# yang-song/score_sde_pytorch

Hardware: NVIDIA H100
Metric: PC-sampler images/sec, NCSN++ CIFAR-10 1000-step VE (higher is better)
Workload: dtype f16 operands (11-bit significand, as tf32), f32 accumulate and activations

## Files before the change

include/scoresde_b200.h:

```cpp
#ifndef SCORESDE_B200_H_
#define SCORESDE_B200_H_

#ifdef __cplusplus
extern "C" {
#endif

#define B200_API __attribute__((visibility("default")))

B200_API const char* b200_last_error(void);
B200_API int b200_version(void);
B200_API int b200_device_sm_count(int* out);

B200_API int b200_upfirdn2d_f32(const float* x, const float* kernel_host, float* y,
                                int major, int in_h, int in_w, int minor, int kh, int kw,
                                int up_x, int up_y, int down_x, int down_y,
                                int pad_x0, int pad_x1, int pad_y0, int pad_y1, void* stream);

B200_API int b200_fused_bias_act_f32(const float* x, const float* b, const float* ref, float* y,
                                     long long n, int step_b, int size_b, int act, int grad,
                                     float alpha, float scale, void* stream);

B200_API int b200_groupnorm_nhwc_f32(const float* x1, int c1, const float* x2, int c2,
                                     const float* gamma, const float* beta, int batch, int hw, int groups,
                                     float eps, int silu, int round_tf32,
                                     float* stats_ws ,
                                     float* y, float* raw_or_null, void* stream);
B200_API int b200_softmax_rows_f32(const float* s, float* p, long long rows, int t, float scale,
                                   int round_tf32, void* stream);
B200_API int b200_randn_like_torch_f32(float* out, long long numel, unsigned long long seed,
                                       unsigned long long offset, unsigned long long* offset_inc_out,
                                       unsigned long long* offset_ws_dev , void* stream);

B200_API int b200_conv_nhwc_f32(const float* x1, int c1, const float* x2, int c2, int batch, int h, int w,
                                const float* w_packed, const float* bias, int c_out, int ksize,
                                const float* rowvec, long long rowvec_ld, const float* residual, float scale,
                                int round_tf32, float* out, int impl, void* stream);
B200_API int b200_conv_skip_nhwc_f32(const float* x, int c, const float* s1, int cs1, const float* s2, int cs2,
                                     int batch, int h, int w, const float* w_packed, const float* bias,
                                     const float* w_skip, const float* bias_skip, int c_out, const float* residual,
                                     float scale, int round_tf32, float* out, void* stream);
B200_API int b200_pack_conv_weight_f32(const float* w_oihw, float* w_packed, int c_out, int c_in, int ksize,
                                       int round_tf32, void* stream);
B200_API int b200_attention_core_f32(const float* qk, const float* vT, const float* w3, const float* bv,
                                     const float* b3, const float* x, float* out, double* qstats, int nimg,
                                     int t, int c, float out_scale, int operand_f16, void* stream);
B200_API int b200_gemm_nt_f32(const float* a, long long lda, int a_batch_rows, const float* w, long long ldw,
                              int w_batch_rows, int nbatch, int m, int n, int k, const float* bias,
                              int round_tf32, float* out, long long ldo, int impl, void* stream);

typedef struct b200_ncsnpp b200_ncsnpp_t;

typedef struct {
  int image_size, num_channels, nf, num_res_blocks;
  int num_levels;  int ch_mult[8];
  int num_attn_resolutions;  int attn_resolutions[8];
  int centered, scale_by_sigma, skip_rescale, conditional;
  int progressive_input;
  int fir_taps;  float fir_kernel[8];
  int precision;
  int keep_activations;
  int lanes;
  int cuda_core_head;
  int separate_groupnorm;
  int embedding_type;
  int naive_resample;
  int progressive;
  int pdl;
  int no_halo;
  int family;
  int tangent;
} b200_ncsnpp_config;

B200_API int b200_ncsnpp_create(const b200_ncsnpp_config* cfg, b200_ncsnpp_t** out);
B200_API void b200_ncsnpp_destroy(b200_ncsnpp_t* h);
B200_API int b200_ncsnpp_num_params(const b200_ncsnpp_t* h);
B200_API int b200_ncsnpp_param_info(const b200_ncsnpp_t* h, int index, char* name, int name_cap,
                                    long long shape[4], int* ndim);
B200_API long long b200_ncsnpp_weights_bytes(const b200_ncsnpp_t* h);
B200_API int b200_ncsnpp_bind_weights(b200_ncsnpp_t* h, void* blob_dev);
B200_API int b200_ncsnpp_load_param(b200_ncsnpp_t* h, int index, const float* src_dev, void* stream);
B200_API long long b200_ncsnpp_workspace_bytes(b200_ncsnpp_t* h, int batch);
B200_API int b200_ncsnpp_bind_workspace(b200_ncsnpp_t* h, int batch, void* ws_dev, long long ws_bytes);
B200_API int b200_ncsnpp_forward(b200_ncsnpp_t* h, const float* x_nchw, const float* labels,
                                 int labels_uniform, float* out_nchw, void* stream);
B200_API int b200_ncsnpp_tap(b200_ncsnpp_t* h, int module_index, float* dst_nchw, long long dst_cap_elems,
                             int shape_out[4], void* stream);
B200_API long long b200_ncsnpp_launches_per_forward(const b200_ncsnpp_t* h);
B200_API int b200_ncsnpp_jvp(b200_ncsnpp_t* h, const float* x_nchw, const float* labels, int labels_uniform,
                             const float* v_nchw, float* out_nchw, float* jvp_out_nchw, void* stream);
B200_API int b200_ncsnpp_tap_tangent(b200_ncsnpp_t* h, int module_index, float* dst_nchw, long long dst_cap_elems,
                                     int shape_out[4], void* stream);
B200_API int b200_ncsnpp_profile_forward(b200_ncsnpp_t* h, const float* x_nchw, const float* labels,
                                         int labels_uniform, float* out_nchw, void* stream,
// ... 58 lines not shown
```

score_sde_pytorch_b200/_lib.py:

```python
import ctypes
import os
import threading

from . import build as _build

_LOCK = threading.Lock()
_LIB = None

c_void_p, c_int, c_ll, c_ull, c_float = (ctypes.c_void_p, ctypes.c_int, ctypes.c_longlong,
                                         ctypes.c_ulonglong, ctypes.c_float)
c_char_p = ctypes.c_char_p
P = ctypes.POINTER


class NcsnppConfig(ctypes.Structure):
  _fields_ = [('image_size', c_int), ('num_channels', c_int), ('nf', c_int), ('num_res_blocks', c_int),
              ('num_levels', c_int), ('ch_mult', c_int * 8),
              ('num_attn_resolutions', c_int), ('attn_resolutions', c_int * 8),
              ('centered', c_int), ('scale_by_sigma', c_int), ('skip_rescale', c_int), ('conditional', c_int),
              ('progressive_input', c_int),
              ('fir_taps', c_int), ('fir_kernel', c_float * 8),
              ('precision', c_int), ('keep_activations', c_int), ('lanes', c_int),
              ('cuda_core_head', c_int), ('separate_groupnorm', c_int),
              ('embedding_type', c_int), ('naive_resample', c_int), ('progressive', c_int), ('pdl', c_int),
              ('no_halo', c_int), ('family', c_int), ('tangent', c_int)]


class PcConfig(ctypes.Structure):
  _fields_ = [('n_steps', c_int), ('corrector', c_int), ('predictor', c_int), ('n_corrector_steps', c_int),
              ('snr', c_float),
              ('label', P(c_float)), ('score_scale', P(c_float)), ('alpha', P(c_float)),
              ('pa', P(c_float)), ('pb', P(c_float)), ('pc', P(c_float)),
              ('ca', P(c_float)), ('cb', P(c_float)), ('cc', P(c_float)),
              ('constraint', c_int), ('cm', P(c_float)), ('cs', P(c_float)),
              ('color_m', c_float * 9), ('color_minv', c_float * 9), ('noise_nhwc', c_int)]


SIGNATURES = {
  'b200_last_error': (c_char_p, []),
  'b200_version': (c_int, []),
  'b200_device_sm_count': (c_int, [P(c_int)]),
  'b200_upfirdn2d_f32': (c_int, [c_void_p, P(c_float), c_void_p] + [c_int] * 14 + [c_void_p]),
  'b200_fused_bias_act_f32': (c_int, [c_void_p, c_void_p, c_void_p, c_void_p, c_ll, c_int, c_int, c_int, c_int,
                                      c_float, c_float, c_void_p]),
  'b200_groupnorm_nhwc_f32': (c_int, [c_void_p, c_int, c_void_p, c_int, c_void_p, c_void_p, c_int, c_int, c_int,
                                      c_float, c_int, c_int, c_void_p, c_void_p, c_void_p, c_void_p]),
  'b200_softmax_rows_f32': (c_int, [c_void_p, c_void_p, c_ll, c_int, c_float, c_int, c_void_p]),
  'b200_randn_like_torch_f32': (c_int, [c_void_p, c_ll, c_ull, c_ull, P(c_ull), c_void_p, c_void_p]),
  'b200_conv_nhwc_f32': (c_int, [c_void_p, c_int, c_void_p, c_int, c_int, c_int, c_int, c_void_p, c_void_p, c_int,
                                 c_int, c_void_p, c_ll, c_void_p, c_float, c_int, c_void_p, c_int, c_void_p]),
  'b200_conv_skip_nhwc_f32': (c_int, [c_void_p, c_int, c_void_p, c_int, c_void_p, c_int, c_int, c_int, c_int, c_void_p,
                                      c_void_p, c_void_p, c_void_p, c_int, c_void_p, c_float, c_int, c_void_p, c_void_p]),
  'b200_attention_core_f32': (c_int, [c_void_p, c_void_p, c_void_p, c_void_p, c_void_p, c_void_p, c_void_p, c_void_p,
                                      c_int, c_int, c_int, c_float, c_int, c_void_p]),
  'b200_pack_conv_weight_f32': (c_int, [c_void_p, c_void_p, c_int, c_int, c_int, c_int, c_void_p]),
  'b200_gemm_nt_f32': (c_int, [c_void_p, c_ll, c_int, c_void_p, c_ll, c_int, c_int, c_int, c_int, c_int, c_void_p,
                               c_int, c_void_p, c_ll, c_int, c_void_p]),
  'b200_ncsnpp_create': (c_int, [P(NcsnppConfig), P(c_void_p)]),
  'b200_ncsnpp_destroy': (None, [c_void_p]),
  'b200_ncsnpp_num_params': (c_int, [c_void_p]),
  'b200_ncsnpp_param_info': (c_int, [c_void_p, c_int, c_char_p, c_int, P(c_ll), P(c_int)]),
  'b200_ncsnpp_weights_bytes': (c_ll, [c_void_p]),
  'b200_ncsnpp_bind_weights': (c_int, [c_void_p, c_void_p]),
  'b200_ncsnpp_load_param': (c_int, [c_void_p, c_int, c_void_p, c_void_p]),
  'b200_ncsnpp_num_ops': (c_ll, [c_void_p]),
  'b200_ncsnpp_op_info': (c_int, [c_void_p, c_ll, c_char_p, c_int, P(c_int), P(ctypes.c_double)]),
  'b200_ncsnpp_op_bytes': (c_int, [c_void_p, c_ll, P(ctypes.c_double)]),
  'b200_ncsnpp_profile_ops': (c_int, [c_void_p, c_void_p, c_void_p, c_int, c_void_p, c_void_p, c_void_p, c_ll]),
  'b200_ncsnpp_workspace_bytes': (c_ll, [c_void_p, c_int]),
  'b200_ncsnpp_bind_workspace': (c_int, [c_void_p, c_int, c_void_p, c_ll]),
  'b200_ncsnpp_forward': (c_int, [c_void_p, c_void_p, c_void_p, c_int, c_void_p, c_void_p]),
  'b200_ncsnpp_tap': (c_int, [c_void_p, c_int, c_void_p, c_ll, P(c_int), c_void_p]),
  'b200_ncsnpp_launches_per_forward': (c_ll, [c_void_p]),
  'b200_ncsnpp_jvp': (c_int, [c_void_p, c_void_p, c_void_p, c_int, c_void_p, c_void_p, c_void_p, c_void_p]),
  'b200_ncsnpp_tap_tangent': (c_int, [c_void_p, c_int, c_void_p, c_ll, P(c_int), c_void_p]),
  'b200_ncsnpp_profile_forward': (c_int, [c_void_p, c_void_p, c_void_p, c_int, c_void_p, c_void_p,
                                          P(c_float), P(ctypes.c_double), P(c_ll)]),
  'b200_pc_create': (c_int, [c_void_p, P(PcConfig), c_int, P(c_void_p)]),
  'b200_pc_destroy': (None, [c_void_p]),
  'b200_pc_workspace_bytes': (c_ll, [c_void_p]),
  'b200_pc_bind_workspace': (c_int, [c_void_p, c_void_p, c_ll, c_void_p]),
  'b200_pc_run': (c_int, [c_void_p, c_void_p, c_void_p, c_int, c_int, c_ull, c_ull, P(c_ull), c_int, c_void_p]),
  'b200_pc_bind_constraint': (c_int, [c_void_p, c_void_p, c_void_p, c_void_p]),
  'b200_pc_step_external': (c_int, [c_void_p, c_void_p, c_void_p, c_int, c_void_p, c_void_p, c_void_p]),
  'b200_pc_launches_per_step': (c_ll, [c_void_p]),
  'b200_ode_stage_f64': (c_int, [c_void_p, c_void_p, c_ll, P(ctypes.c_double), c_int, ctypes.c_double, c_void_p, c_void_p, c_void_p]),
  'b200_ode_drift_f64': (c_int, [c_void_p, c_void_p, c_ll, c_void_p, c_void_p, c_void_p]),
  'b200_ode_div_f64': (c_int, [c_void_p, c_void_p, c_int, c_ll, c_void_p, c_void_p, c_void_p]),
  'b200_ode_workspace_doubles': (c_ll, []),
  'b200_ode_error_sumsq_f64': (c_int, [c_void_p, c_void_p, c_void_p, c_ll, P(ctypes.c_double), c_int, ctypes.c_double,
                                       ctypes.c_double, ctypes.c_double, c_void_p, c_void_p]),
  'b200_ode_scaled_sumsq_f64': (c_int, [c_void_p, c_void_p, c_void_p, c_ll, ctypes.c_double, ctypes.c_double, c_void_p, c_void_p]),
  'b200_dsm_perturb_f32': (c_int, [c_void_p, c_void_p, c_void_p, c_void_p, c_void_p, c_int, c_ll, c_void_p]),
  'b200_dsm_workspace_doubles': (c_ll, [c_int, c_ll]),
  'b200_dsm_loss_f32': (c_int, [c_void_p, c_void_p, c_void_p, c_void_p, c_void_p, c_int, c_ll, c_int, c_int, c_void_p, c_void_p]),
}


def library_path():
  return _build.LIB


def load():
  global _LIB
  with _LOCK:
# ... 32 lines not shown
```

score_sde_pytorch_b200/csrc/api.cu:

```cuda
#include "kernels.h"
#include "../../include/scoresde_b200.h"
#include <cstring>

namespace b200 {
namespace { thread_local bool tl_pdl = false; }
bool pdl_active() { return tl_pdl; }
PdlScope::PdlScope(bool on) : prev(tl_pdl) { tl_pdl = on; }
PdlScope::~PdlScope() { tl_pdl = prev; }


static thread_local char g_err[1024] = "";

void set_error(const char* fmt, ...) {
  va_list ap;
  va_start(ap, fmt);
  vsnprintf(g_err, sizeof(g_err), fmt, ap);
  va_end(ap);
}
const char* last_error() { return g_err; }

}

using namespace b200;

// ... 63 lines not shown
}

int b200_conv_nhwc_f32(const float* x1, int c1, const float* x2, int c2, int batch, int h, int w,
                       const float* w_packed, const float* bias, int c_out, int ksize, const float* rowvec,
                       long long rowvec_ld, const float* residual, float scale, int round_tf32, float* out, int impl,
                       void* stream) {
  B200_REQUIRE(x1 && w_packed && out, "conv_nhwc: null pointer");
  B200_REQUIRE(ksize == 1 || ksize == 3, "conv_nhwc: ksize %d unsupported", ksize);
  cudaStream_t st = static_cast<cudaStream_t>(stream);
  Epilogue ep; memset(&ep, 0, sizeof(ep));
  ep.bias = bias; ep.rowvec = rowvec; ep.rowvec_ld = rowvec_ld; ep.residual = residual; ep.ld_res = c_out;
  ep.scale = scale; ep.round_tf32 = round_tf32; ep.rows_per_img = h * w; ep.out = out; ep.ld_out = c_out;
  if (!x2) c2 = 0;
  if (impl == 1 || impl == 2 || impl == 4 || impl == 5) {
    TcGemmDesc d; memset(&d, 0, sizeof(d));
    d.f16 = impl == 2 || impl == 5; d.no_halo = impl >= 4 ? 1 : 0;
    d.a1 = x1; d.C1 = c1; d.a2 = x2; d.C2 = c2; d.conv = 1; d.H = h; d.W = w; d.nimg = batch; d.taps = ksize * ksize;
    d.w = w_packed; d.N_total = c_out; d.K_total = c1 + c2; d.w_rows = (long long)ksize * ksize * c_out; d.nbatch = 1;
    d.epi = ep;
    TcGemmPlan* pl = nullptr;
    if (int r = tc_gemm_plan_create(d, &pl)) return r;
    const int r = tc_gemm_launch(pl, st);
    tc_gemm_plan_destroy(pl);
    return r;
  }
  SimtConv s; memset(&s, 0, sizeof(s));
  s.x1 = x1; s.C1 = c1; s.x2 = x2; s.C2 = c2; s.in_scale = 1.f; s.H = h; s.W = w; s.R = s.S = ksize; s.stride = 1;
  s.pad = ksize / 2; s.OH = h; s.OW = w; s.nbatch = batch; s.a_batched = 1; s.w = w_packed; s.N = c_out; s.epi = ep;
  if (impl == 3) return launch_conv_lowc(s, st);
  B200_REQUIRE(impl == 0, "conv_nhwc: impl %d unknown", impl);
  return launch_conv_simt(s, st);
}

int b200_conv_skip_nhwc_f32(const float* x, int c, const float* s1, int cs1, const float* s2, int cs2, int batch, int h,
                            int w, const float* w_packed, const float* bias, const float* w_skip,
                            const float* bias_skip, int c_out, const float* residual, float scale, int round_tf32,
                            float* out, void* stream) {
  B200_REQUIRE(x && s1 && w_packed && w_skip && out, "conv_skip_nhwc: null pointer");
  Epilogue ep; memset(&ep, 0, sizeof(ep));
  ep.bias = bias; ep.rowvec = bias_skip; ep.rowvec_ld = 0; ep.residual = residual; ep.ld_res = c_out;
  ep.scale = scale; ep.round_tf32 = round_tf32; ep.rows_per_img = h * w; ep.out = out; ep.ld_out = c_out;
  TcGemmDesc d; memset(&d, 0, sizeof(d));
  d.a1 = x; d.C1 = c; d.conv = 1; d.H = h; d.W = w; d.nimg = batch; d.taps = 9;
  d.w = w_packed; d.N_total = c_out; d.K_total = c; d.w_rows = 9LL * c_out; d.nbatch = 1;
  d.a3 = s1; d.C3 = cs1; d.a4 = s2; d.C4 = s2 ? cs2 : 0; d.w2 = w_skip;
  d.epi = ep;
  TcGemmPlan* pl = nullptr;
  if (int r = tc_gemm_plan_create(d, &pl)) return r;
  const int r = tc_gemm_launch(pl, static_cast<cudaStream_t>(stream));
  tc_gemm_plan_destroy(pl);
  return r;
}

int b200_attention_core_f32(const float* qk, const float* vT, const float* w3, const float* bv, const float* b3,
                            const float* x, float* out, double* qstats, int nimg, int t, int c, float out_scale,
                            int operand_f16, void* stream) {
  B200_REQUIRE(tc_attn_supported(t, c), "attention_core: only T=256, C=256 is implemented (got T=%d C=%d)", t, c);
  TcAttnDesc d; memset(&d, 0, sizeof(d));
  d.qk = qk; d.vT = vT; d.w3 = w3; d.bv = bv; d.b3 = b3; d.x = x; d.out = out; d.qstats = qstats;
  d.nimg = nimg; d.T = t; d.C = c; d.out_scale = out_scale; d.f16 = operand_f16 ? 1 : 0;
  TcAttnPlan* pl = nullptr;
  if (int r = tc_attn_plan_create(d, &pl)) return r;
  const int r = tc_attn_launch(pl, static_cast<cudaStream_t>(stream));
  tc_attn_plan_destroy(pl);
  return r;
}

int b200_gemm_nt_f32(const float* a, long long lda, int a_batch_rows, const float* w, long long ldw, int w_batch_rows,
                     int nbatch, int m, int n, int k, const float* bias, int round_tf32, float* out, long long ldo,
                     int impl, void* stream) {
  B200_REQUIRE(a && w && out && nbatch > 0, "gemm_nt: bad argument");
  cudaStream_t st = static_cast<cudaStream_t>(stream);
  Epilogue ep; memset(&ep, 0, sizeof(ep));
  ep.bias = bias; ep.scale = 1.f; ep.round_tf32 = round_tf32; ep.rows_per_img = m; ep.out = out; ep.ld_out = ldo;
  if (impl == 1 || impl == 2) {
    TcGemmDesc d; memset(&d, 0, sizeof(d));
    d.f16 = impl == 2;
    d.a1 = a; d.C1 = k; d.conv = 0; d.taps = 1; d.a_ld = lda; d.a_batch_rows = a_batch_rows;
    d.a_rows = a_batch_rows ? (long long)a_batch_rows * (nbatch - 1) + m : m;
    d.w = w; d.N_total = n; d.K_total = k; d.w_ld = ldw; d.w_batch_rows = w_batch_rows;
    d.w_rows = w_batch_rows ? (long long)w_batch_rows * (nbatch - 1) + n : n;
    d.nbatch = nbatch; d.M_per_batch = m; d.epi = ep;
    TcGemmPlan* pl = nullptr;
    if (int r = tc_gemm_plan_create(d, &pl)) return r;
    const int r = tc_gemm_launch(pl, st);
    tc_gemm_plan_destroy(pl);
    return r;
  }
  SimtConv s; memset(&s, 0, sizeof(s));
  s.x1 = a; s.C1 = k; s.ld1 = lda; s.in_scale = 1.f; s.H = m; s.W = 1; s.R = s.S = 1; s.stride = 1; s.pad = 0;
  s.OH = m; s.OW = 1; s.nbatch = nbatch; s.a_batched = a_batch_rows != 0; s.w = w; s.N = n;
  s.w_batch_stride = (long long)w_batch_rows * ldw; s.w_ld = ldw; s.epi = ep;
  B200_REQUIRE(!a_batch_rows || a_batch_rows == m, "gemm_nt(simt): a_batch_rows must be 0 or m");
  return launch_conv_simt(s, st);
}

}
```

score_sde_pytorch_b200/csrc/gemm_tc.cu:

```cuda
#include "kernels.h"
#include <cuda.h>
#include <cudaTypedefs.h>
#include <cuda_fp16.h>
#include "wgmma.cuh"
#include <mutex>
#include <cstdlib>
#include <cstring>

namespace b200 {

namespace {

constexpr int BM = 128;
constexpr int BKE = 32;
constexpr int A_STAGE_BYTES = BM * BKE * 4;

constexpr int HALO_XS = 4;
constexpr int HALO_X_BYTES = 40 * 1024;
constexpr int HALO_WS = 4;

struct TcParams {
  CUtensorMap tmA1, tmA2, tmW;
  CUtensorMap tmA3, tmA4, tmW2;
  CUtensorMap tmH1, tmH2;
  int halo;
  int halo_dh_bytes;
  int halo_copy_bytes;
  int halo_prefetch;
  int chunk_major;
  int conv, H, W, taps, pad, S, stride;
  int kchunks1, kchunks2, C1;
  int kchunks3, kchunks4, C3;
  int N_total, tiles_n;
  int nbatch, tiles_m_per_batch, M_per_batch;
  int a_batch_rows, w_batch_rows;
  int f16;
  int bke;
  int swap;
  double* qstats;
  long long total_tiles;
  Epilogue epi;
};

__device__ __forceinline__ uint32_t smem_u32(const void* p) { return (uint32_t)__cvta_generic_to_shared(p); }

__device__ __forceinline__ void mbar_init(uint64_t* bar, uint32_t count) {
  asm volatile("mbarrier.init.shared::cta.b64 [%0], %1;" ::"r"(smem_u32(bar)), "r"(count));
}
__device__ __forceinline__ void mbar_expect_tx(uint64_t* bar, uint32_t bytes) {
  asm volatile("mbarrier.arrive.expect_tx.shared::cta.b64 _, [%0], %1;" ::"r"(smem_u32(bar)), "r"(bytes) : "memory");
}
__device__ __forceinline__ void mbar_arrive(uint64_t* bar) {
  asm volatile("mbarrier.arrive.shared::cta.b64 _, [%0];" ::"r"(smem_u32(bar)) : "memory");
}
__device__ __forceinline__ bool mbar_try_wait(uint64_t* bar, uint32_t parity) {
  uint32_t ok;
  asm volatile(
      "{\n\t.reg .pred p;\n\t"
      "mbarrier.try_wait.parity.shared::cta.b64 p, [%1], %2;\n\t"
      "selp.u32 %0, 1, 0, p;\n\t}"
      : "=r"(ok) : "r"(smem_u32(bar)), "r"(parity) : "memory");
  return ok != 0;
}
__device__ __forceinline__ void mbar_wait(uint64_t* bar, uint32_t parity) {
  if (mbar_try_wait(bar, parity)) return;
  const long long t0 = clock64();
  while (!mbar_try_wait(bar, parity)) {
    if (clock64() - t0 > 8000000000LL) __trap();
  }
}

__device__ __forceinline__ void tma_load_4d(const CUtensorMap* tm, void* dst, uint64_t* bar, int c0, int c1, int c2, int c3) {
  asm volatile(
      "cp.async.bulk.tensor.4d.shared::cluster.global.mbarrier::complete_tx::bytes [%0], [%1, {%3, %4, %5, %6}], [%2];"
      ::"r"(smem_u32(dst)), "l"(tm), "r"(smem_u32(bar)), "r"(c0), "r"(c1), "r"(c2), "r"(c3) : "memory");
}
__device__ __forceinline__ void tma_load_2d(const CUtensorMap* tm, void* dst, uint64_t* bar, int c0, int c1) {
  asm volatile(
      "cp.async.bulk.tensor.2d.shared::cluster.global.mbarrier::complete_tx::bytes [%0], [%1, {%3, %4}], [%2];"
      ::"r"(smem_u32(dst)), "l"(tm), "r"(smem_u32(bar)), "r"(c0), "r"(c1) : "memory");
}

__device__ __forceinline__ void tma_prefetch_4d(const CUtensorMap* tm, int c0, int c1, int c2, int c3) {
  asm volatile("cp.async.bulk.prefetch.tensor.4d.L2.global.tile [%0, {%1, %2, %3, %4}];" ::"l"(tm), "r"(c0), "r"(c1), "r"(c2), "r"(c3) : "memory");
}

__device__ __forceinline__ void fence_async_smem() { asm volatile("fence.proxy.async.shared::cta;" ::: "memory"); }

__device__ __forceinline__ uint64_t make_smem_desc(uint32_t saddr) {
  return (uint64_t)((saddr & 0x3FFFFu) >> 4) | (1ull << 16) | ((uint64_t)(1024 >> 4) << 32) | (1ull << 62);
}

template <int N, bool F16>
__device__ __forceinline__ void wgmma_kstep(float (&d)[N / 2], uint64_t adesc, uint64_t bdesc, int it) {
  wgmma_fence();
#pragma unroll
  for (int k = 0; k < 4; ++k) {
    const uint32_t acc = (it | k) != 0;
    if constexpr (F16) {
      if constexpr (N == 256) wgmma_f16_n256(d, adesc + 2 * k, bdesc + 2 * k, acc);
      else wgmma_f16_n128(d, adesc + 2 * k, bdesc + 2 * k, acc);
    } else {
      if constexpr (N == 256) wgmma_tf32_n256(d, adesc + 2 * k, bdesc + 2 * k, acc);
      else wgmma_tf32_n128(d, adesc + 2 * k, bdesc + 2 * k, acc);
    }
  }
  wgmma_commit();
}

__device__ __forceinline__ bool elect_one() {
  uint32_t pred;
  asm volatile("{\n\t.reg .pred p;\n\telect.sync _|p, 0xffffffff;\n\tselp.u32 %0, 1, 0, p;\n\t}" : "=r"(pred));
  return pred != 0;
}
__device__ __forceinline__ void regs_producer() { asm volatile("setmaxnreg.dec.sync.aligned.u32 40;"); }
__device__ __forceinline__ void regs_consumer() { asm volatile("setmaxnreg.inc.sync.aligned.u32 232;"); }
__device__ __forceinline__ void wg_barrier(int g) { asm volatile("bar.sync %0, 128;" ::"r"(g + 1) : "memory"); }

template <int BN>
struct SmemLayout {
  static constexpr int STAGES = BN == 256 ? 4 : 6;
  static constexpr int B_STAGE_BYTES = BN * BKE * 4;
  static constexpr int STAGE_BYTES = A_STAGE_BYTES + B_STAGE_BYTES;
  static constexpr int RING_BYTES = STAGES * STAGE_BYTES;
  static constexpr int HALO_BYTES = HALO_XS * HALO_X_BYTES + HALO_WS * A_STAGE_BYTES;
  static constexpr int BAR_OFFSET = BN == 256 && HALO_BYTES > RING_BYTES ? HALO_BYTES : RING_BYTES;
  static constexpr int TOTAL = BAR_OFFSET + 256 + 1024;
  static_assert(TOTAL <= 232448, "exceeds the 227 KB shared-memory limit of sm_90");
  static_assert(BN != 256 || STAGES >= HALO_XS, "the halo copies use the first HALO_XS stage barriers");
};

template <int BN, bool RES, int MODE, bool STATS>
__device__ __forceinline__ void frag_rows(const float (&d)[BN / 2], const Epilogue& e, double* qstats, int n_total,
                                          long long gm, int rows_valid, int n0, int lane) {
  const int ra = lane >> 2, rb = ra + 8;
  const bool va = ra < rows_valid, vb = rb < rows_valid;
  const int img = rows_valid > 0 ? (int)gm / e.rows_per_img : 0;
  const float* rv = e.rowvec ? e.rowvec + (long long)img * e.rowvec_ld : nullptr;
  const float scale = e.scale;
#pragma unroll
  for (int j = 0; j < BN / 8; ++j) {
    const int col = n0 + 8 * j + 2 * (lane & 3);
    float2 ad = make_float2(0.f, 0.f);
    if (e.bias) ad = __ldg(reinterpret_cast<const float2*>(e.bias + col));
    if (rv) { const float2 t = __ldg(reinterpret_cast<const float2*>(rv + col)); ad.x += t.x; ad.y += t.y; }
    float o0 = d[4 * j] + ad.x, o1 = d[4 * j + 1] + ad.y, o2 = d[4 * j + 2] + ad.x, o3 = d[4 * j + 3] + ad.y;
    if (RES) {
      if (va) { const float2 r = __ldg(reinterpret_cast<const float2*>(e.residual + (gm + ra) * e.ld_res + col)); o0 += r.x; o1 += r.y; }
      if (vb) { const float2 r = __ldg(reinterpret_cast<const float2*>(e.residual + (gm + rb) * e.ld_res + col)); o2 += r.x; o3 += r.y; }
    }
    o0 *= scale; o1 *= scale; o2 *= scale; o3 *= scale;
    if (MODE == 1) { o0 = round_tf32(o0); o1 = round_tf32(o1); o2 = round_tf32(o2); o3 = round_tf32(o3); }
    if (MODE == 2) {
      uint16_t* oh = reinterpret_cast<uint16_t*>(e.out);
      if (va) *reinterpret_cast<uint32_t*>(oh + (gm + ra) * e.ld_out + col) = pack_half2(o0, o1);
      if (vb) *reinterpret_cast<uint32_t*>(oh + (gm + rb) * e.ld_out + col) = pack_half2(o2, o3);
    } else {
      if (va) *reinterpret_cast<float2*>(e.out + (gm + ra) * e.ld_out + col) = make_float2(o0, o1);
      if (vb) *reinterpret_cast<float2*>(e.out + (gm + rb) * e.ld_out + col) = make_float2(o2, o3);
    }
    if (STATS) {
      float s = (va ? o0 + o1 : 0.f) + (vb ? o2 + o3 : 0.f);
      float q = (va ? fmaf(o0, o0, o1 * o1) : 0.f) + (vb ? fmaf(o2, o2, o3 * o3) : 0.f);
#pragma unroll
      for (int m = 4; m <= 16; m <<= 1) { s += __shfl_xor_sync(0xffffffffu, s, m); q += __shfl_xor_sync(0xffffffffu, q, m); }
      s += __shfl_xor_sync(0xffffffffu, s, 1); q += __shfl_xor_sync(0xffffffffu, q, 1);
      if ((lane & ~2) == 0 && rows_valid > 0) {
        double* qd = qstats + ((long long)img * (n_total >> 2) + (col >> 2)) * 2;
        atomicAdd(qd, (double)s); atomicAdd(qd + 1, (double)q);
      }
    }
  }
}
template <int BN>
__device__ __forceinline__ void frag_rows_dispatch(const float (&d)[BN / 2], const Epilogue& e, double* qstats, int n_total,
                                                   long long gm, int rows_valid, int n0, int lane) {
  const int mode = e.round_tf32;
  const bool has_res = e.residual != nullptr, stats = qstats != nullptr;
#define B200_ROWF(R, M) do { if (stats) frag_rows<BN, R, M, true>(d, e, qstats, n_total, gm, rows_valid, n0, lane); \
                             else frag_rows<BN, R, M, false>(d, e, qstats, n_total, gm, rows_valid, n0, lane); } while (0)
  if (has_res) { if (mode == 0) B200_ROWF(true, 0); else if (mode == 1) B200_ROWF(true, 1); else B200_ROWF(true, 2); }
  else { if (mode == 0) B200_ROWF(false, 0); else if (mode == 1) B200_ROWF(false, 1); else B200_ROWF(false, 2); }
#undef B200_ROWF
}

template <bool RES, int MODE, bool STATS>
__device__ __forceinline__ void frag_swap(const float (&d)[128], const Epilogue& e, double* qstats, int n_total,
                                          int c0, long long pix0, int img, int lane) {
  const int ca = c0 + (lane >> 2), cb = ca + 8;
  const float adda = (e.bias ? __ldg(e.bias + ca) : 0.f) + (e.rowvec ? __ldg(e.rowvec + img * e.rowvec_ld + ca) : 0.f);
  const float addb = (e.bias ? __ldg(e.bias + cb) : 0.f) + (e.rowvec ? __ldg(e.rowvec + img * e.rowvec_ld + cb) : 0.f);
  const float scale = e.scale;
  float sa = 0.f, qa = 0.f, sb = 0.f, qb = 0.f;
#pragma unroll
  for (int j = 0; j < 32; ++j) {
    const long long px = pix0 + 8 * j + 2 * (lane & 3);
    float o[4] = {d[4 * j] + adda, d[4 * j + 1] + adda, d[4 * j + 2] + addb, d[4 * j + 3] + addb};
#pragma unroll
    for (int i = 0; i < 4; ++i) {
      const long long pix = px + (i & 1);
      const int ch = i < 2 ? ca : cb;
      if (RES) o[i] += __ldg(e.residual + pix * e.ld_res + ch);
      o[i] *= scale;
      if (MODE == 1) o[i] = round_tf32(o[i]);
      if (MODE == 2) {
        uint16_t h;
        asm("cvt.rn.f16.f32 %0, %1;" : "=h"(h) : "f"(o[i]));
        reinterpret_cast<uint16_t*>(e.out)[pix * e.ld_out + ch] = h;
      } else e.out[pix * e.ld_out + ch] = o[i];
    }
    if (STATS) {
      sa += o[0] + o[1]; qa = fmaf(o[0], o[0], fmaf(o[1], o[1], qa));
      sb += o[2] + o[3]; qb = fmaf(o[2], o[2], fmaf(o[3], o[3], qb));
    }
  }
  if (STATS) {
#pragma unroll
    for (int m = 1; m <= 8; m <<= 1) {
      sa += __shfl_xor_sync(0xffffffffu, sa, m); qa += __shfl_xor_sync(0xffffffffu, qa, m);
      sb += __shfl_xor_sync(0xffffffffu, sb, m); qb += __shfl_xor_sync(0xffffffffu, qb, m);
    }
    if ((lane & 15) == 0) {
      double* qd = qstats + ((long long)img * (n_total >> 2) + (ca >> 2)) * 2;
      atomicAdd(qd, (double)sa); atomicAdd(qd + 1, (double)qa);
      qd = qstats + ((long long)img * (n_total >> 2) + (cb >> 2)) * 2;
      atomicAdd(qd, (double)sb); atomicAdd(qd + 1, (double)qb);
    }
  }
}

template <int BN, bool F16>
__device__ __forceinline__ void gemm_tc_consumer(const TcParams& p, uint8_t* smem, uint64_t* full_bar, uint64_t* empty_bar,
                                                 uint64_t* wfull_bar, uint64_t* wempty_bar, int g, int wq, int lane) {
  using L = SmemLayout<BN>;
  const int kiters = (p.kchunks1 + p.kchunks2) * p.taps + p.kchunks3 + p.kchunks4;
  const Epilogue& e = p.epi;
  uint32_t stage = 0, phase = 0, ws = 0, wphase = 0;
  for (int tile = blockIdx.x; tile < p.total_tiles; tile += gridDim.x) {
    float acc[BN / 2];
    if (BN == 256 && p.halo) {
      const uint32_t wring = smem_u32(smem + HALO_XS * HALO_X_BYTES);
      int it = 0, pend_ws = -1, pend_x = -1;
      for (int src = 0; src < 4; ++src) {
        const int nch = src == 0 ? p.kchunks1 : src == 1 ? p.kchunks2 : src == 2 ? p.kchunks3 : p.kchunks4;
        const int ncopies = src < 2 ? 3 * nch : nch, ntap = src < 2 ? 3 : 1;
        for (int c = 0; c < ncopies; ++c) {
          mbar_wait(&full_bar[stage], phase);
          const uint32_t sx = smem_u32(smem + stage * HALO_X_BYTES);
          for (int dhi = 0; dhi < ntap; ++dhi, ++it) {
            mbar_wait(&wfull_bar[ws], wphase);
            const uint64_t adesc = make_smem_desc(wring + ws * A_STAGE_BYTES + g * (A_STAGE_BYTES / 2));
            const uint64_t bdesc = make_smem_desc(sx + (src < 2 ? dhi * p.halo_dh_bytes : 0));
            wgmma_kstep<BN, F16>(acc, adesc, bdesc, it);
            wgmma_wait<1>();
            if (lane == 0) {
              if (pend_ws >= 0) mbar_arrive(&wempty_bar[pend_ws]);
              if (pend_x >= 0) mbar_arrive(&empty_bar[pend_x]);
            }
            pend_ws = (int)ws; pend_x = dhi == ntap - 1 ? (int)stage : -1;
            if (++ws == HALO_WS) { ws = 0; wphase ^= 1; }
          }
          if (++stage == HALO_XS) { stage = 0; phase ^= 1; }
        }
      }
      wgmma_wait<0>();
      if (lane == 0) {
        if (pend_ws >= 0) mbar_arrive(&wempty_bar[pend_ws]);
        if (pend_x >= 0) mbar_arrive(&empty_bar[pend_x]);
      }
    } else {
      int pend = -1;
      for (int it = 0; it < kiters; ++it) {
        mbar_wait(&full_bar[stage], phase);
        const uint32_t sa = smem_u32(smem + stage * L::STAGE_BYTES);
        wgmma_kstep<BN, F16>(acc, make_smem_desc(sa + g * (A_STAGE_BYTES / 2)), make_smem_desc(sa + A_STAGE_BYTES), it);
        wgmma_wait<1>();
        if (lane == 0 && pend >= 0) mbar_arrive(&empty_bar[pend]);
        pend = (int)stage;
        if (++stage == L::STAGES) { stage = 0; phase ^= 1; }
      }
      wgmma_wait<0>();
      if (lane == 0 && pend >= 0) mbar_arrive(&empty_bar[pend]);
    }

    const int rw = g * 64 + wq * 16;
    if constexpr (BN == 256) {
      if (p.swap) {
        const int c0 = (int)(tile % p.tiles_n) * 128 + rw;
        const int pix0 = (tile / p.tiles_n) * 256;
        const int img = pix0 / e.rows_per_img;
        if (e.out_nchw) {
          const float dv = e.per_img_div ? __ldg(e.per_img_div + img * e.div_stride) : 1.f;
          const int hw = e.rows_per_img, pix_in_img = (int)(pix0 - (long long)img * hw);
#pragma unroll
          for (int h = 0; h < 2; ++h) {
            const int co = c0 + (lane >> 2) + 8 * h;
            if (co < e.n_valid) {
              const float add = e.bias ? __ldg(e.bias + co) : 0.f;
              float* dst = e.out + ((long long)img * e.n_valid + co) * hw + pix_in_img + 2 * (lane & 3);
#pragma unroll
              for (int j = 0; j < 32; ++j)
                *reinterpret_cast<float2*>(dst + 8 * j) = make_float2((acc[4 * j + 2 * h] + add) / dv, (acc[4 * j + 2 * h + 1] + add) / dv);
            }
          }
        } else {
          const int mode = e.round_tf32;
          const bool has_res = e.residual != nullptr, stats = p.qstats != nullptr;
#define B200_SWAPF(R, M) do { if (stats) frag_swap<R, M, true>(acc, e, p.qstats, p.N_total, c0, pix0, img, lane); \
                              else frag_swap<R, M, false>(acc, e, p.qstats, p.N_total, c0, pix0, img, lane); } while (0)
          if (has_res) { if (mode == 0) B200_SWAPF(true, 0); else if (mode == 1) B200_SWAPF(true, 1); else B200_SWAPF(true, 2); }
          else { if (mode == 0) B200_SWAPF(false, 0); else if (mode == 1) B200_SWAPF(false, 1); else B200_SWAPF(false, 2); }
#undef B200_SWAPF
        }
        continue;
      }
    }
    const int nt = (int)(tile % p.tiles_n);
    const int mg = tile / p.tiles_n;
    const int b = (int)(mg / p.tiles_m_per_batch);
    const int mt = (int)(mg % p.tiles_m_per_batch);
    const int row0 = mt * BM + rw;
    const int rows_valid = min(16, max(0, p.M_per_batch - row0));
    frag_rows_dispatch<BN>(acc, e, p.qstats, p.N_total, (long long)b * p.M_per_batch + row0, rows_valid, nt * BN, lane);
  }
}

template <int BN>
__global__ void __launch_bounds__(384, 1) gemm_tc_kernel(const __grid_constant__ TcParams p) {
  using L = SmemLayout<BN>;
  constexpr int STAGES = L::STAGES;
  extern __shared__ uint8_t smem_raw[];
  uint8_t* smem = reinterpret_cast<uint8_t*>((reinterpret_cast<uintptr_t>(smem_raw) + 1023) & ~uintptr_t(1023));
  uint64_t* full_bar = reinterpret_cast<uint64_t*>(smem + L::BAR_OFFSET);
  uint64_t* empty_bar = full_bar + STAGES;
  uint64_t* wfull_bar = empty_bar + STAGES;
  uint64_t* wempty_bar = wfull_bar + HALO_WS;

  const int warp = __shfl_sync(0xffffffffu, threadIdx.x >> 5, 0), lane = threadIdx.x & 31;

  if (threadIdx.x == 0) {
    for (int s = 0; s < STAGES; ++s) { mbar_init(&full_bar[s], 1); mbar_init(&empty_bar[s], 8); }
    for (int s = 0; s < HALO_WS; ++s) { mbar_init(&wfull_bar[s], 1); mbar_init(&wempty_bar[s], 8); }
    asm volatile("fence.mbarrier_init.release.cluster;" ::: "memory");
    asm volatile("fence.proxy.async.shared::cta;" ::: "memory");
  }
  __syncthreads();
  pdl_wait(); pdl_trigger();

  const int HW = p.H * p.W;
  const int bke = p.bke;

  if (warp < 4) {
    regs_producer();
    if (warp != 0) return;
    const bool issue = elect_one();
    uint32_t stage = 0, phase = 0;
    if (BN == 256 && p.halo) {
      uint32_t ws = 0, wphase = 0;
      uint8_t* const wring = smem + HALO_XS * HALO_X_BYTES;
      for (int tile = blockIdx.x; tile < p.total_tiles; tile += gridDim.x) {
        const int nt = (int)(tile % p.tiles_n);
        const int p0 = (tile / p.tiles_n) * 256;
// ... 169 lines not shown
    if (d.nbatch != 1) return fail("conv mode is unbatched");
    if (d.stride > 2) return fail("stride must be 1 or 2");
    if (d.stride == 2 && d.a2) return fail("strided conv is single-source");
    const int HW = d.H * d.W;
    if (HW >= BM) {
      if (d.W >= BM) { if (d.W % BM) return fail("image width does not tile 128 pixels"); }
      else if ((BM % d.W) || (d.H % (BM / d.W))) return fail("image rows do not tile 128 pixels");
    } else if (BM % HW) return fail("image size does not divide 128 pixels");
  } else {
    if (d.nbatch > 1 && (d.M_per_batch % BM)) return fail("batched gemm needs M_per_batch % 128 == 0");
    if (d.a_ld % (d.f16 ? 8 : 4)) return fail("A row pitch must be a multiple of 16 bytes");
  }
  if (d.a3) {
    if (!d.conv || d.stride == 2 || !d.w2) return fail("extra 1x1 phase needs a stride-1 convolution and its weights");
    if (d.C3 % bke || d.C3 <= 0 || (d.a4 && d.C4 % bke)) return fail("extra-phase channel counts must be multiples of 32 (tf32) / 64 (f16)");
  }
  if (d.epi.out_nchw) {
    if (!(d.conv && d.N_total == 128 && d.epi.n_valid > 0 && d.epi.n_valid <= 32 && (d.H * d.W) % 256 == 0 && (d.W <= BM || d.W % BM == 0) && d.stride != 2 &&
          !d.qstats && !d.epi.residual && !d.epi.rowvec && d.epi.round_tf32 == 0))
      return fail("NCHW head needs a 128-row padded weight tile, HW % 256 == 0 and a plain epilogue");
  } else if (d.epi.per_img_div) return fail("per-image divisor only with the NCHW head epilogue");
  if ((d.qstats || d.epi.rowvec) && !(d.epi.rows_per_img % 32 == 0 || d.epi.rows_per_img == 16)) return fail("per-image epilogue terms need rows_per_img % 32 == 0 or == 16");
  if (d.epi.ld_out % 4 || (d.epi.residual && d.epi.ld_res % 4)) return fail("output pitch must be a multiple of 4 elements");
  if (d.epi.round_tf32 == 2 && d.epi.ld_out % 8) return fail("fp16 output pitch must be a multiple of 8 elements");
  return true;
}

int tc_gemm_plan_create(const TcGemmDesc& d, TcGemmPlan** out) {
  const char* why = nullptr;
  B200_REQUIRE(tc_gemm_supported(d, &why), "gemm_tc: unsupported shape: %s", why ? why : "?");
  if (int r = tc_configure()) return r;
  TcGemmPlan* pl = new TcGemmPlan();
  TcParams& p = pl->prm;
  memset(&p, 0, sizeof(p));
  pl->bn = (d.N_total % 256 == 0) ? 256 : 128;
  p.conv = d.conv; p.H = d.conv ? d.H : 1; p.W = d.conv ? d.W : 1; p.taps = d.taps;
  p.S = d.taps == 9 ? 3 : 1; p.pad = (d.taps == 9 && !d.valid_pad) ? 1 : 0;
  p.stride = d.stride == 2 ? 2 : 1;
  p.f16 = d.f16 ? 1 : 0;

  const bool f16 = d.f16 != 0;
  const int bke = f16 ? 64 : BKE;
  const uint64_t es = f16 ? 2 : 4;
  p.bke = bke;
  {
    const long long Mtot = (long long)d.nimg * d.H * d.W;
    const bool halo_geom = d.taps == 9 && p.pad == 1 && (d.W == 16 || d.W == 32) && (d.Hin == 0 || d.Hin == d.H) &&
                           (d.Win == 0 || d.Win == d.W);
    const bool can_swap = d.conv && p.stride == 1 && (d.N_total % 256 != 0 || d.taps == 1 || halo_geom) && (d.H * d.W) % 256 == 0 &&
                          (d.W <= BM || d.W % BM == 0) && Mtot % 256 == 0 && d.epi.rows_per_img % 256 == 0;
    p.swap = can_swap ? 1 : 0;
    if (d.epi.out_nchw && !p.swap) { delete pl; B200_REQUIRE(false, "gemm_tc: the NCHW head needs the swapped-operand form"); }
    if (p.swap) pl->bn = 256;
    p.qstats = d.qstats;
    const int tmb = d.conv ? 1 : (d.M_per_batch + BM - 1) / BM;
    const long long m_tiles = d.conv ? (Mtot + BM - 1) / BM : (long long)d.nbatch * tmb;
    const long long n_tiles = d.N_total % 256 == 0 ? d.N_total / 256 : d.N_total / 128;
    if (!p.swap && pl->bn == 256 && m_tiles * n_tiles <= num_sms() / 2) pl->bn = 128;
  }
  p.kchunks1 = d.C1 / bke; p.kchunks2 = d.a2 ? d.C2 / bke : 0; p.C1 = d.C1;
  p.N_total = d.N_total; p.tiles_n = p.swap ? d.N_total / 128 : d.N_total / pl->bn;
  p.a_batch_rows = d.a_batch_rows; p.w_batch_rows = d.w_batch_rows;
  p.epi = d.epi;

  int rc = 0;
  if (d.conv) {
    const int HW = d.H * d.W;
    const long long M = (long long)d.nimg * HW;
    p.nbatch = 1; p.M_per_batch = (int)M; p.tiles_m_per_batch = p.swap ? (int)(M / 256) : (int)((M + BM - 1) / BM);
    uint32_t box[4];
    if (HW >= BM) { box[1] = std::min(d.W, BM); box[2] = BM / box[1]; box[3] = 1; }
    else { box[1] = d.W; box[2] = d.H; box[3] = BM / HW; }
    box[0] = (uint32_t)bke;
    const uint32_t estr[4] = {1, (uint32_t)p.stride, (uint32_t)p.stride, 1};
    box[1] *= p.stride; box[2] *= p.stride;
    const int Hin = d.Hin ? d.Hin : d.H, Win = d.Win ? d.Win : d.W;
    for (int s = 0; s < 2; ++s) {
      const float* base = s ? d.a2 : d.a1;
      const int C = s ? d.C2 : d.C1;
      if (!base) continue;
      uint64_t dims[4] = {(uint64_t)C, (uint64_t)Win, (uint64_t)Hin, (uint64_t)d.nimg};
      uint64_t str[3] = {(uint64_t)C * es, (uint64_t)Win * C * es, (uint64_t)Hin * Win * C * es};
      rc = encode_map(s ? &p.tmA2 : &p.tmA1, base, 4, dims, str, box, estr, f16);
      if (rc) { delete pl; return rc; }
    }
  } else {
    p.nbatch = d.nbatch; p.M_per_batch = d.M_per_batch; p.tiles_m_per_batch = (d.M_per_batch + BM - 1) / BM;
    uint32_t box[4] = {(uint32_t)bke, BM, 1, 1};
    for (int s = 0; s < 2; ++s) {
      const float* base = s ? d.a2 : d.a1;
      if (!base) continue;
      uint64_t dims[4] = {(uint64_t)(s ? d.C2 : d.C1), (uint64_t)d.a_rows, 1, 1};
      uint64_t str[3] = {(uint64_t)d.a_ld * es, (uint64_t)d.a_ld * es * d.a_rows, (uint64_t)d.a_ld * es * d.a_rows};
      rc = encode_map(s ? &p.tmA2 : &p.tmA1, base, 4, dims, str, box, nullptr, f16);
      if (rc) { delete pl; return rc; }
    }
  }
  if (!d.a2) p.tmA2 = p.tmA1;
  p.tmA3 = p.tmA1; p.tmA4 = p.tmA1;
  p.tmH1 = p.tmA1; p.tmH2 = p.tmA1;
  {
    const int tile_px = p.swap ? 256 : BM;
    const bool halo = (d.no_halo & 3) != 1 && d.conv && d.taps == 9 && p.pad == 1 && p.stride == 1 && p.swap &&
                      (d.W == 16 || d.W == 32) && (d.H * d.W) % tile_px == 0 && (d.Hin == 0 || d.Hin == d.H) && (d.Win == 0 || d.Win == d.W);
    const bool halo_shape = d.conv && d.taps == 9 && p.pad == 1 && p.stride == 1 && (d.W == 16 || d.W == 32) && (d.H * d.W) % tile_px == 0 &&
                            (d.Hin == 0 || d.Hin == d.H) && (d.Win == 0 || d.Win == d.W);
// ... 142 lines not shown
```

Measured before the change: 8.249.

## Stage swapped-conv epilogue through shared memory with cp.async residual prefetch

```diff
diff --git a/include/scoresde_b200.h b/include/scoresde_b200.h
--- a/include/scoresde_b200.h
+++ b/include/scoresde_b200.h
@@ -39,6 +39,11 @@
                                      int batch, int h, int w, const float* w_packed, const float* bias,
                                      const float* w_skip, const float* bias_skip, int c_out, const float* residual,
                                      float scale, int round_tf32, float* out, void* stream);
+B200_API int b200_conv_tc_qstats_nhwc_f32(const float* x1, int c1, const float* x2, int c2, const float* s1, int cs1,
+                                          const float* s2, int cs2, int batch, int h, int w, const float* w_packed,
+                                          const float* bias, const float* w_skip, int c_out, const float* rowvec,
+                                          long long rowvec_ld, const float* residual, float scale, int round_tf32,
+                                          float* out, double* qstats, int f16, void* stream);
 B200_API int b200_pack_conv_weight_f32(const float* w_oihw, float* w_packed, int c_out, int c_in, int ksize,
                                        int round_tf32, void* stream);
 B200_API int b200_attention_core_f32(const float* qk, const float* vT, const float* w3, const float* bv,
diff --git a/score_sde_pytorch_b200/_lib.py b/score_sde_pytorch_b200/_lib.py
--- a/score_sde_pytorch_b200/_lib.py
+++ b/score_sde_pytorch_b200/_lib.py
@@ -51,6 +51,9 @@
                                  c_int, c_void_p, c_ll, c_void_p, c_float, c_int, c_void_p, c_int, c_void_p]),
   'b200_conv_skip_nhwc_f32': (c_int, [c_void_p, c_int, c_void_p, c_int, c_void_p, c_int, c_int, c_int, c_int, c_void_p,
                                       c_void_p, c_void_p, c_void_p, c_int, c_void_p, c_float, c_int, c_void_p, c_void_p]),
+  'b200_conv_tc_qstats_nhwc_f32': (c_int, [c_void_p, c_int, c_void_p, c_int, c_void_p, c_int, c_void_p, c_int, c_int, c_int,
+                                           c_int, c_void_p, c_void_p, c_void_p, c_int, c_void_p, c_ll, c_void_p, c_float,
+                                           c_int, c_void_p, c_void_p, c_int, c_void_p]),
   'b200_attention_core_f32': (c_int, [c_void_p, c_void_p, c_void_p, c_void_p, c_void_p, c_void_p, c_void_p, c_void_p,
                                       c_int, c_int, c_int, c_float, c_int, c_void_p]),
   'b200_pack_conv_weight_f32': (c_int, [c_void_p, c_void_p, c_int, c_int, c_int, c_int, c_void_p]),
diff --git a/score_sde_pytorch_b200/csrc/api.cu b/score_sde_pytorch_b200/csrc/api.cu
--- a/score_sde_pytorch_b200/csrc/api.cu
+++ b/score_sde_pytorch_b200/csrc/api.cu
@@ -139,6 +139,29 @@
   return r;
 }
 
+int b200_conv_tc_qstats_nhwc_f32(const float* x1, int c1, const float* x2, int c2, const float* s1, int cs1,
+                                 const float* s2, int cs2, int batch, int h, int w, const float* w_packed,
+                                 const float* bias, const float* w_skip, int c_out, const float* rowvec,
+                                 long long rowvec_ld, const float* residual, float scale, int round_tf32,
+                                 float* out, double* qstats, int f16, void* stream) {
+  B200_REQUIRE(x1 && w_packed && out && (!s1 || w_skip), "conv_tc_qstats_nhwc: null pointer");
+  Epilogue ep; memset(&ep, 0, sizeof(ep));
+  ep.bias = bias; ep.rowvec = rowvec; ep.rowvec_ld = rowvec_ld; ep.residual = residual; ep.ld_res = c_out;
+  ep.scale = scale; ep.round_tf32 = round_tf32; ep.rows_per_img = h * w; ep.out = out; ep.ld_out = c_out;
+  TcGemmDesc d; memset(&d, 0, sizeof(d));
+  d.f16 = f16 ? 1 : 0;
+  d.a1 = x1; d.C1 = c1; d.a2 = x2; d.C2 = x2 ? c2 : 0; d.conv = 1; d.H = h; d.W = w; d.nimg = batch; d.taps = 9;
+  d.w = w_packed; d.N_total = c_out; d.K_total = c1 + d.C2; d.w_rows = 9LL * c_out; d.nbatch = 1;
+  if (s1) { d.a3 = s1; d.C3 = cs1; d.a4 = s2; d.C4 = s2 ? cs2 : 0; d.w2 = w_skip; }
+  d.qstats = qstats;
+  d.epi = ep;
+  TcGemmPlan* pl = nullptr;
+  if (int r = tc_gemm_plan_create(d, &pl)) return r;
+  const int r = tc_gemm_launch(pl, static_cast<cudaStream_t>(stream));
+  tc_gemm_plan_destroy(pl);
+  return r;
+}
+
 int b200_attention_core_f32(const float* qk, const float* vT, const float* w3, const float* bv, const float* b3,
                             const float* x, float* out, double* qstats, int nimg, int t, int c, float out_scale,
                             int operand_f16, void* stream) {
diff --git a/score_sde_pytorch_b200/csrc/gemm_tc.cu b/score_sde_pytorch_b200/csrc/gemm_tc.cu
--- a/score_sde_pytorch_b200/csrc/gemm_tc.cu
+++ b/score_sde_pytorch_b200/csrc/gemm_tc.cu
@@ -15,9 +15,14 @@
 constexpr int BKE = 32;
 constexpr int A_STAGE_BYTES = BM * BKE * 4;
 
-constexpr int HALO_XS = 4;
+constexpr int HALO_XS = 3;
 constexpr int HALO_X_BYTES = 40 * 1024;
 constexpr int HALO_WS = 4;
+
+constexpr int EPI_PX = 8, EPI_PITCH = 20, EPI_NBUF = 6;
+constexpr int EPI_CHUNK = EPI_PX * EPI_PITCH;
+constexpr int EPI_WARP_FLOATS = EPI_NBUF * EPI_CHUNK;
+constexpr int EPI_BYTES = 8 * EPI_WARP_FLOATS * 4;
 
 struct TcParams {
   CUtensorMap tmA1, tmA2, tmW;
@@ -87,6 +92,24 @@
 
 __device__ __forceinline__ void fence_async_smem() { asm volatile("fence.proxy.async.shared::cta;" ::: "memory"); }
 
+__device__ __forceinline__ void cp_async16(uint32_t dst, const void* src) {
+  asm volatile("cp.async.cg.shared.global [%0], [%1], 16;" ::"r"(dst), "l"(src) : "memory");
+}
+__device__ __forceinline__ void cp_async_commit() { asm volatile("cp.async.commit_group;" ::: "memory"); }
+template <int N>
+__device__ __forceinline__ void cp_async_wait() { asm volatile("cp.async.wait_group %0;" ::"n"(N) : "memory"); }
+__device__ __forceinline__ float lds_f32(uint32_t a) {
+  float v;
+  asm volatile("ld.shared.f32 %0, [%1];" : "=f"(v) : "r"(a) : "memory");
+  return v;
+}
+__device__ __forceinline__ void sts_f32(uint32_t a, float v) { asm volatile("st.shared.f32 [%0], %1;" ::"r"(a), "f"(v) : "memory"); }
+__device__ __forceinline__ float4 lds_f32x4(uint32_t a) {
+  float4 v;
+  asm volatile("ld.shared.v4.f32 {%0, %1, %2, %3}, [%4];" : "=f"(v.x), "=f"(v.y), "=f"(v.z), "=f"(v.w) : "r"(a) : "memory");
+  return v;
+}
+
 __device__ __forceinline__ uint64_t make_smem_desc(uint32_t saddr) {
   return (uint64_t)((saddr & 0x3FFFFu) >> 4) | (1ull << 16) | ((uint64_t)(1024 >> 4) << 32) | (1ull << 62);
 }
@@ -124,7 +147,8 @@
   static constexpr int STAGE_BYTES = A_STAGE_BYTES + B_STAGE_BYTES;
   static constexpr int RING_BYTES = STAGES * STAGE_BYTES;
   static constexpr int HALO_BYTES = HALO_XS * HALO_X_BYTES + HALO_WS * A_STAGE_BYTES;
-  static constexpr int BAR_OFFSET = BN == 256 && HALO_BYTES > RING_BYTES ? HALO_BYTES : RING_BYTES;
+  static constexpr int EPI_OFFSET = BN == 256 && HALO_BYTES > RING_BYTES ? HALO_BYTES : RING_BYTES;
+  static constexpr int BAR_OFFSET = EPI_OFFSET + (BN == 256 ? EPI_BYTES : 0);
   static constexpr int TOTAL = BAR_OFFSET + 256 + 1024;
   static_assert(TOTAL <= 232448, "exceeds the 227 KB shared-memory limit of sm_90");
   static_assert(BN != 256 || STAGES >= HALO_XS, "the halo copies use the first HALO_XS stage barriers");
@@ -184,9 +208,19 @@
 #undef B200_ROWF
 }
 
+__device__ __forceinline__ void res_chunk_copy(uint32_t buf, const Epilogue& e, long long pix, int c0, int lane) {
+  const int px = lane >> 2, part = lane & 3;
+  cp_async16(buf + 4 * (px * EPI_PITCH + 4 * part), e.residual + (pix + px) * e.ld_res + c0 + 4 * part);
+}
+
+__device__ __forceinline__ void res_stage_begin(uint32_t stage, const Epilogue& e, int c0, long long pix0, int lane) {
+#pragma unroll
+  for (int k = 0; k < EPI_NBUF; ++k) { res_chunk_copy(stage + 4 * k * EPI_CHUNK, e, pix0 + EPI_PX * k, c0, lane); cp_async_commit(); }
+}
+
 template <bool RES, int MODE, bool STATS>
 __device__ __forceinline__ void frag_swap(const float (&d)[128], const Epilogue& e, double* qstats, int n_total,
-                                          int c0, long long pix0, int img, int lane) {
+                                          int c0, long long pix0, int img, uint32_t stage, int lane) {
   const int ca = c0 + (lane >> 2), cb = ca + 8;
   const float adda = (e.bias ? __ldg(e.bias + ca) : 0.f) + (e.rowvec ? __ldg(e.rowvec + img * e.rowvec_ld + ca) : 0.f);
   const float addb = (e.bias ? __ldg(e.bias + cb) : 0.f) + (e.rowvec ? __ldg(e.rowvec + img * e.rowvec_ld + cb) : 0.f);
@@ -194,20 +228,26 @@
   float sa = 0.f, qa = 0.f, sb = 0.f, qb = 0.f;
 #pragma unroll
   for (int j = 0; j < 32; ++j) {
-    const long long px = pix0 + 8 * j + 2 * (lane & 3);
+    const uint32_t buf = stage + 4 * (j % EPI_NBUF) * EPI_CHUNK;
+    if (RES) { cp_async_wait<EPI_NBUF - 1>(); __syncwarp(); }
     float o[4] = {d[4 * j] + adda, d[4 * j + 1] + adda, d[4 * j + 2] + addb, d[4 * j + 3] + addb};
 #pragma unroll
     for (int i = 0; i < 4; ++i) {
-      const long long pix = px + (i & 1);
-      const int ch = i < 2 ? ca : cb;
-      if (RES) o[i] += __ldg(e.residual + pix * e.ld_res + ch);
+      const uint32_t s = buf + 4 * ((2 * (lane & 3) + (i & 1)) * EPI_PITCH + (lane >> 2) + (i < 2 ? 0 : 8));
+      if (RES) o[i] += lds_f32(s);
       o[i] *= scale;
       if (MODE == 1) o[i] = round_tf32(o[i]);
-      if (MODE == 2) {
-        uint16_t h;
-        asm("cvt.rn.f16.f32 %0, %1;" : "=h"(h) : "f"(o[i]));
-        reinterpret_cast<uint16_t*>(e.out)[pix * e.ld_out + ch] = h;
-      } else e.out[pix * e.ld_out + ch] = o[i];
+      sts_f32(s, o[i]);
+    }
+    __syncwarp();
+    const float4 v = lds_f32x4(buf + 4 * ((lane >> 2) * EPI_PITCH + 4 * (lane & 3)));
+    const long long at = (pix0 + EPI_PX * j + (lane >> 2)) * e.ld_out + c0 + 4 * (lane & 3);
+    if (MODE == 2) *reinterpret_cast<uint2*>(reinterpret_cast<uint16_t*>(e.out) + at) = make_uint2(pack_half2(v.x, v.y), pack_half2(v.z, v.w));
+    else *reinterpret_cast<float4*>(e.out + at) = v;
+    if (RES) {
+      __syncwarp();
+      if (j + EPI_NBUF < 32) res_chunk_copy(buf, e, pix0 + EPI_PX * (j + EPI_NBUF), c0, lane);
+      cp_async_commit();
     }
     if (STATS) {
       sa += o[0] + o[1]; qa = fmaf(o[0], o[0], fmaf(o[1], o[1], qa));
@@ -237,6 +277,9 @@
   const Epilogue& e = p.epi;
   uint32_t stage = 0, phase = 0, ws = 0, wphase = 0;
   for (int tile = blockIdx.x; tile < p.total_tiles; tile += gridDim.x) {
+    if (BN == 256 && p.swap && e.residual)
+      res_stage_begin(smem_u32(smem + L::EPI_OFFSET) + 4 * (g * 4 + wq) * EPI_WARP_FLOATS, e,
+                      (int)(tile % p.tiles_n) * 128 + g * 64 + wq * 16, (tile / p.tiles_n) * 256LL, lane);
     float acc[BN / 2];
     if (BN == 256 && p.halo) {
       const uint32_t wring = smem_u32(smem + HALO_XS * HALO_X_BYTES);
@@ -304,10 +347,11 @@
             }
           }
         } else {
+          const uint32_t epi_stage = smem_u32(smem + L::EPI_OFFSET) + 4 * (g * 4 + wq) * EPI_WARP_FLOATS;
           const int mode = e.round_tf32;
           const bool has_res = e.residual != nullptr, stats = p.qstats != nullptr;
-#define B200_SWAPF(R, M) do { if (stats) frag_swap<R, M, true>(acc, e, p.qstats, p.N_total, c0, pix0, img, lane); \
-                              else frag_swap<R, M, false>(acc, e, p.qstats, p.N_total, c0, pix0, img, lane); } while (0)
+#define B200_SWAPF(R, M) do { if (stats) frag_swap<R, M, true>(acc, e, p.qstats, p.N_total, c0, pix0, img, epi_stage, lane); \
+                              else frag_swap<R, M, false>(acc, e, p.qstats, p.N_total, c0, pix0, img, epi_stage, lane); } while (0)
           if (has_res) { if (mode == 0) B200_SWAPF(true, 0); else if (mode == 1) B200_SWAPF(true, 1); else B200_SWAPF(true, 2); }
           else { if (mode == 0) B200_SWAPF(false, 0); else if (mode == 1) B200_SWAPF(false, 1); else B200_SWAPF(false, 2); }
 #undef B200_SWAPF
@@ -583,6 +627,9 @@
     p.swap = can_swap ? 1 : 0;
     if (d.epi.out_nchw && !p.swap) { delete pl; B200_REQUIRE(false, "gemm_tc: the NCHW head needs the swapped-operand form"); }
     if (p.swap) pl->bn = 256;
+    if (p.swap && !d.epi.out_nchw && ((reinterpret_cast<uintptr_t>(d.epi.out) | reinterpret_cast<uintptr_t>(d.epi.residual)) & 15)) {
+      delete pl; B200_REQUIRE(false, "gemm_tc: the swapped epilogue needs 16-byte-aligned output and residual");
+    }
     p.qstats = d.qstats;
     const int tmb = d.conv ? 1 : (d.M_per_batch + BM - 1) / BM;
     const long long m_tiles = d.conv ? (Mtot + BM - 1) / BM : (long long)d.nbatch * tmb;
```

Result: faster. 8.612, median of 6 (+4.4%).
